# barry-mir/mixing-style-transfer

Measured on AMD Instinct MI355X. Metric: triplets/sec (10 s @ 44.1 kHz, 4-stem, bs=24), higher is better.
Workload: dtype f32

## Files before the change

mixing-style-transfer_amd/csrc/encoder.hip:

```cpp
#include "common.h"

#include <cmath>
#include <type_traits>
#include <vector>

namespace {

typedef float f32x4 __attribute__((ext_vector_type(4)));
constexpr int kConvThreads = 512;
constexpr int kConvWaves = 8;

struct FilmParams {
  const float* feats;
  const float *w0t, *b0, *w3t, *b3, *hwt, *hb;
  const float *s1, *t1, *s2, *t2;
  float* film;
  float2* aff1;
  float2* aff2;
  int Fd, H, nsub;
  float* h2;
  int B;
};

constexpr int kFilmCT = 8;
// ... 97 lines not shown
      p.aff2[((size_t)b * p.nsub + band) * 64 + c2] = make_float2(g * p.s2[band * 64 + c2], fmaf(g, p.t2[band * 64 + c2], be));
    }
  }
}

constexpr size_t film_lds_bytes(int Fd, int H) {
  return (size_t)((Fd + H) * kFilmCT + 5 * kFilmCT * 64) * sizeof(float);
}
hipError_t launch_film(const FilmParams& fp, hipStream_t st) {
  const int tiles = (fp.B + kFilmCT - 1) / kFilmCT;
  const size_t lds_h = (size_t)((fp.Fd + fp.H) * kFilmCT + 4 * kFilmCT * 64) * sizeof(float);
  const size_t lds_o = (size_t)(fp.H * kFilmCT + 5 * kFilmCT * 64) * sizeof(float);
  hipLaunchKernelGGL(film_hidden_kernel, dim3(tiles, (fp.H + 63) / 64), dim3(256), lds_h, st, fp);
  hipLaunchKernelGGL(film_head_kernel, dim3(tiles, fp.nsub * 3), dim3(256), lds_o, st, fp);
  return hipGetLastError();
}

template <int LAYER, int SUB>
struct CC;
template <int SUB>
struct CC<1, SUB> {
  static constexpr int CIN = 8, COUT = 32, NCH = 2, MT = 5, NT = 2;
  static constexpr int WIN = 5 * SUB;
  static constexpr int WPG = 20 / WIN;
  static constexpr int TROWS = SUB, TCOLS = 5 * 4 * WPG;
  static constexpr int PR = TROWS + 6, PC = TCOLS + 6;
  static constexpr int RL = PC <= 64 ? 64 : 128;
};
template <int SUB>
struct CC<2, SUB> {
  static constexpr int CIN = 32, COUT = 64, NCH = 8, MT = 4, NT = 4;
  static constexpr int WIN = 16, WPG = 1;
  static constexpr int TROWS = 8, TCOLS = 8;
  static constexpr int PR = 14, PC = 14;
  static constexpr int RL = 16;
};

template <int SUB>
struct CC<3, SUB> {
  static constexpr int CIN = 64, COUT = 32, NCH = 16, MT = 5, NT = 2;
  static constexpr int WIN = 10, WPG = 2;
  static constexpr int TROWS = 2, TCOLS = 40;
  static constexpr int PR = TROWS + 6, PC = TCOLS + 6;
  static constexpr int RL = 64;
};

template <int SUB>
struct CC<4, SUB> {
  static constexpr int CIN = 32, COUT = 64, NCH = 8, MT = 5, NT = 4;
  static constexpr int WIN = 10, WPG = 2;
  static constexpr int TROWS = 2, TCOLS = 40;
  static constexpr int PR = TROWS + 6, PC = TCOLS + 6;
  static constexpr int RL = 64;
};

struct ConvParams {
  const float* in;
  const float* wfrag;
  const float2* aff;
  float* out;
  int B, nsub;
  int in_rows, in_cols;
  int in_cstride;
  int in_bandoff;
  long long in_clipstride;
  int out_rows, out_cols;
  int tiles_r, tiles_c;
  int sets_per_band;
  float* yraw;
  mst::DetAcc* stats;
  const float* bias;
  int raw_rows, raw_cols;
  const unsigned char* mask;
  float mask_scale;
  int acc_tr, acc_tc, row_off;
  const float* f16_scale;
  const float* f16_winv;
  int pool_h;
  int clip_major;
  _Float16* yraw16;
  const float* y_scale;
  const void* in_lo;
  int cm_mels, cm_overlap;
};

typedef _Float16 h16x4 __attribute__((ext_vector_type(4)));
__device__ __forceinline__ size_t yvec(size_t unit, int t, int nvec) {
  return (unit & ~(size_t)63) * nvec + (size_t)t * 64 + (unit & 63);
}
template <int NV>
__device__ __forceinline__ void load_unit(const void* yraw, const float* y_scale, int band, size_t unit, float (&v)[NV]) {
  if (y_scale) {
    const float inv = y_scale[band * 2 + 1];
    const h16x4* s = reinterpret_cast<const h16x4*>(yraw);
#pragma unroll
    for (int t = 0; t < NV / 4; ++t) {
      const h16x4 q = s[yvec(unit, t, NV / 4)];
#pragma unroll
      for (int r = 0; r < 4; ++r) v[4 * t + r] = (float)q[r] * inv;
    }
  } else {
    const f32x4* s = reinterpret_cast<const f32x4*>(yraw);
#pragma unroll
    for (int t = 0; t < NV / 4; ++t) {
      const f32x4 q = s[yvec(unit, t, NV / 4)];
#pragma unroll
      for (int r = 0; r < 4; ++r) v[4 * t + r] = q[r];
    }
  }
}

template <int NT, int COUT>
__device__ __forceinline__ void flush_stats(double (&st)[NT][2], mst::DetAcc* stats, int band, int lane) {
#pragma unroll
  for (int n = 0; n < NT; ++n)
#pragma unroll
    for (int k = 0; k < 2; ++k) {
      double x = st[n][k];
      x += __shfl_xor(x, 16, 64);
      x += __shfl_xor(x, 32, 64);
      if (lane < 16) mst::det_add(&stats[((size_t)band * COUT + n * 16 + lane) * 2 + k], x);
      st[n][k] = 0.0;
    }
}

struct Tile {
  int valid, clip, band, tr, tc;
};

template <class F, int... I>
__device__ __forceinline__ void static_for_impl(F&& f, std::integer_sequence<int, I...>) {
  (f(std::integral_constant<int, I>{}), ...);
}
template <int N, class F>
__device__ __forceinline__ void static_for(F&& f) {
  static_for_impl(f, std::make_integer_sequence<int, N>{});
}


template <int LAYER, int SUB>
struct ConvGeom {
  using C = CC<LAYER, SUB>;
  static constexpr int WCH = 49 * C::NT * 64;
  static constexpr int NWF = (WCH / 4 + kConvThreads - 1) / kConvThreads;
  static constexpr int WBP = NWF * kConvThreads * 4;
  static constexpr int PATCH = (4 * C::PR * C::PC + 3) / 4 * 4;
  static constexpr int NPF = (4 * C::PR * C::RL + 63) / 64;
  static constexpr int NCV = C::RL >= 64 ? C::RL / 64 : 1;
};

template <int LAYER, int SUB, int MODE = 0>
__global__ __launch_bounds__(kConvThreads) void conv_kernel(const ConvParams p) {
  using C = CC<LAYER, SUB>;
  using GEO = ConvGeom<LAYER, SUB>;
  static_assert(MODE == 0 || (MODE == 1 && LAYER <= 2) || (MODE == 2 && LAYER == 3) || (MODE == 3 && LAYER == 4),
                "raw modes: forward layers, conv2 dgrad, conv2 strip");
  constexpr bool GEO1 = LAYER == 1 || LAYER >= 3;
  constexpr int MT = C::MT, NT = C::NT, NCH = C::NCH, PR = C::PR, PC = C::PC, RL = C::RL;
  constexpr int WBP = GEO::WBP, PATCH = GEO::PATCH, NWF = GEO::NWF, NPF = GEO::NPF, NCV = GEO::NCV;
  constexpr bool BL = LAYER == 2;
  constexpr int NPFK = BL ? 16 : NPF;
  constexpr int NPIECE = NPFK + NWF, PPT = (NPIECE + 48) / 49;
  extern __shared__ __attribute__((aligned(16))) float smem[];
  const int tid = threadIdx.x, lane = tid & 63;
  const int wave = __builtin_amdgcn_readfirstlane(tid >> 6);
  float* wbuf = smem;
// ... 266 lines not shown
            st[n][0] += (double)v, st[n][1] += (double)v * (double)v;
            const int tr8 = row >> 3, rr = row & 7, tc8 = col >> 3, cc8 = col & 7;
            const int lane8 = 16 * (((rr >> 2) << 1) | (cc8 >> 2)) + j, e8 = 4 * (rr & 3) + (cc8 & 3);
            yplane[(((((size_t)tr8 * p.acc_tc + tc8) * NT + n) * 4 + (e8 >> 2)) * 64 + lane8) * 4 + (e8 & 3)] = v;
          }
        }
      }
    }
    if (MODE == 2 && chunk == NCH - 1 && cur.valid) {
      const int j = lane & 15, g = lane >> 4;
#pragma unroll
      for (int n = 0; n < NT; ++n) {
        const int ch = n * 16 + j;
        float* ob = p.out + (((size_t)cur.clip * p.nsub + cur.band) * C::COUT + ch) * (size_t)p.raw_rows * p.raw_cols;
        const unsigned char* mb = p.mask ? p.mask + (((size_t)cur.clip * p.nsub + cur.band) * C::COUT + ch) * (size_t)p.raw_rows * p.raw_cols
                                         : nullptr;
#pragma unroll
        for (int e = 0; e < 4 * MT; ++e) {
          const int wv = e / C::WIN, pos = e % C::WIN;
          const int row = C::TROWS * cur.tr + pos / 5, col = C::TCOLS * cur.tc + 5 * (C::WPG * g + wv) + pos % 5;
          if (row < p.raw_rows && col < p.raw_cols) {
            const size_t o = (size_t)row * p.raw_cols + col;
            float v = acc[e >> 2][n][e & 3];
            if (mb) v = mb[o] ? v * p.mask_scale : 0.f;
            ob[o] = v;
          }
        }
      }
    }
    if (MODE == 0 && chunk == NCH - 1 && cur.valid) {
      const int j = lane & 15, g = lane >> 4;
      const float2* aff = p.aff + ((size_t)cur.clip * p.nsub + cur.band) * C::COUT;
#pragma unroll
      for (int n = 0; n < NT; ++n) {
        const int ch = n * 16 + j;
        const float2 ac = aff[ch];
        if constexpr (LAYER == 1) {
#pragma unroll
          for (int wv = 0; wv < C::WPG; ++wv) {
            float m = 0.f;
#pragma unroll
            for (int pos = 0; pos < C::WIN; ++pos) {
              const int e = wv * C::WIN + pos;
              m = fmaxf(m, fmaf(acc[e >> 2][n][e & 3], ac.x, ac.y));
            }
            const int pc = 4 * C::WPG * cur.tc + C::WPG * g + wv;
            if (pc < p.out_cols)
              p.out[((((size_t)cur.clip * p.nsub + cur.band) * C::COUT + ch) * p.out_rows + cur.tr) * p.out_cols + pc] = m;
          }
        } else {
          float m = 0.f;
          if constexpr (TS) {
            float m0 = 0.f, m1 = 0.f;
#pragma unroll
            for (int r = 0; r < 4; ++r) {
              m0 = fmaxf(m0, fmaxf(fmaf(acc[0][n][r], ac.x, ac.y), fmaf(acc[1][n][r], ac.x, ac.y)));
              m1 = fmaxf(m1, fmaxf(fmaf(acc[2][n][r], ac.x, ac.y), fmaf(acc[3][n][r], ac.x, ac.y)));
            }
            m0 = fmaxf(m0, __shfl_xor(m0, 32, 64));
            m1 = fmaxf(m1, __shfl_xor(m1, 32, 64));
            m = (g >> 1) ? m1 : m0;
          } else {
#pragma unroll
            for (int t = 0; t < MT; ++t)
#pragma unroll
              for (int r = 0; r < 4; ++r) m = fmaxf(m, fmaf(acc[t][n][r], ac.x, ac.y));
          }
          const int pr = 2 * cur.tr + (g >> 1), pc = 2 * cur.tc + (g & 1);
          if (pr < p.out_rows && pc < p.out_cols)
            p.out[(((size_t)cur.clip * p.nsub + cur.band) * C::COUT + ch) * p.out_rows * p.out_cols +
                  (size_t)pr * p.out_cols + pc] = m;
        }
      }
    }
  }
#ifdef MST_TRACE
  if (MODE == 0 && LAYER == 2 && lane == 0 && p.yraw) {
    float* o = p.yraw + (blockIdx.x * kConvWaves + wave) * 8;
    for (int i = 0; i < 5; ++i) o[i] = (float)trc[i];
    o[5] = (float)(clock64() - trc_start);
  }
#endif
  if ((MODE == 1 || MODE == 3) && st_band >= 0) flush_stats<NT, C::COUT>(st, p.stats, st_band, lane);
}

template <int SUB, int MODE = 0, int LAY = 0>
__global__ __launch_bounds__(kConvThreads) void conv1_resident_kernel(const ConvParams p) {
  using C = CC<1, SUB>;
  constexpr int MT = C::MT, NT = C::NT, PR = C::PR, PC = C::PC;
  static_assert(C::RL == 64, "resident conv1 expects one loader row per instruction");
  static_assert(LAY == 0 || PR == 8, "the channel-minor loader maps lane bits 1..3 to the 8 patch rows");
  constexpr int WCH = 49 * NT * 64;
  constexpr int WBP = ConvGeom<1, SUB>::WBP;
  constexpr int CHS = PR * PC;
  constexpr int PATCH = 8 * CHS;
  constexpr int NPF = LAY == 0 ? 8 * PR : (PC + 3) / 4;
  extern __shared__ __attribute__((aligned(16))) float smem[];
  const int tid = threadIdx.x, lane = tid & 63;
  const int wave = __builtin_amdgcn_readfirstlane(tid >> 6);
  float* wres = smem;
  float* pbuf = smem + 2 * WCH + wave * PATCH;
  constexpr bool DYN = MODE == 0;
  constexpr int kTickets = 16;
  __shared__ unsigned tickets[kTickets];
#ifdef MST_TRACE
  long long trc[5] = {0, 0, 0, 0, 0};
  const long long trc_start = clock64();
#endif

  const int G = gridDim.x;
  const int wg = mst::xcd_remap(blockIdx.x, G);
  const int total_sets = (p.clip_major ? (p.B + p.clip_major - 1) / p.clip_major : 1) * p.nsub * p.sets_per_band;
  const int s_begin = (int)((long long)wg * total_sets / G), s_end = (int)((long long)(wg + 1) * total_sets / G);
  const int tpb = p.tiles_r * p.tiles_c;

  auto decode = [&](int s) __attribute__((always_inline)) {
    Tile t;
    int ti;
    if (p.clip_major) {
      const int ngrp = (p.B + p.clip_major - 1) / p.clip_major;
      const int gb = min(s / p.sets_per_band, ngrp * p.nsub - 1);
      const int idx = (s - gb * p.sets_per_band) * kConvWaves + wave;
      const int grp = gb / p.nsub, c0 = grp * p.clip_major;
      t.band = gb - grp * p.nsub;
      t.valid = (s < s_end) && idx < min(p.clip_major, p.B - c0) * tpb;
      const int cl = t.valid ? idx / tpb : 0;
      t.clip = c0 + cl;
      ti = t.valid ? idx - cl * tpb : 0;
    } else {
      t.band = min(s / p.sets_per_band, p.nsub - 1);
      const int idx = (s - t.band * p.sets_per_band) * kConvWaves + wave;
      t.valid = (s < s_end) && idx < p.B * tpb;
      t.clip = t.valid ? idx / tpb : 0;
      ti = t.valid ? idx - t.clip * tpb : 0;
    }
    t.tc = ti / p.tiles_r;
    t.tr = ti - t.tc * p.tiles_r;
    return t;
  };

  const int kq = lane >> 4, ai = lane & 15, ag = ai >> 2, areg = ai & 3;
  int abase[MT];
#pragma unroll
  for (int t = 0; t < MT; ++t) {
    const int e = 4 * t + areg, wv = e / C::WIN, pos = e % C::WIN;
    abase[t] = kq * CHS + (pos / 5) * PC + 5 * (C::WPG * ag + wv) + pos % 5;
  }

  typename std::conditional<LAY == 0, float, f32x4>::type pf[NPF];
  unsigned long long rowmask = 0;
  bool col_ok = false;
  int coff = 0, nrow0 = 0, nvalid = 0;
  const float* nsrc = p.in;
  bool nfast = false;
  __amdgpu_buffer_rsrc_t nrsrc = __builtin_amdgcn_make_buffer_rsrc(const_cast<float*>(p.in), 0, 0, 0x00020000);
  unsigned nsoff = 0, nvoff = 0;
  static_assert(WBP - WCH >= 4, "the chunk pitch leaves at least 16 zero bytes behind the weights");
  const float* const zero16 = p.wfrag + WCH;
  const int lr = (lane >> 1) & 7, lhalf = lane & 1, lfq = lane >> 4;
  const unsigned frame_bytes = (unsigned)p.cm_mels * 32u;
  auto prefetch_setup = [&](const Tile& t) __attribute__((always_inline)) {
    nrow0 = C::TROWS * t.tr - 3;
    nvalid = t.valid;
    rowmask = 0;
    if constexpr (LAY == 0) {
      const int col0 = C::TCOLS * t.tc - 3, cin = col0 + lane;
// ... 2334 lines not shown
          for (int c = 0; c < 4; ++c) {
            const float a = low ? dyl[((c * 4 + (lane >> 5)) * 64 + (lane & 31)) * 4 + e] : dyl[((c * 4 + (e >> 2)) * 64 + lane) * 4 + (e & 3)];
            acc[c][KF] = __builtin_amdgcn_mfma_f32_16x16x4f32(a, b, acc[c][KF], 0, 0, 0);
          }
        }
      }
    }
    stage(buf ^ 1, pfs, dqs, pms);
    __syncthreads();
  };
  for (int s = s_begin; s < s_end; s += 2) {
    body(s, 0, pfA, dqA, pmA, pfB, dqB, pmB);
    if (s + 1 < s_end) body(s + 1, 1, pfB, dqB, pmB, pfA, dqA, pmA);
  }
  flush(cur_band, cur_chunk);
}

#include "encoder_f16train.inc"

__global__ void sums_to_dbn_kernel(const mst::DetAcc* sums, float* dbn, int n, const float* unscale) {
  const int i = blockIdx.x * blockDim.x + threadIdx.x;
  const double u = unscale ? (double)unscale[1] : 1.0;
  if (i < n) dbn[i] = (float)(mst::det_get(sums[2 * i + 1]) * u), dbn[n + i] = (float)(mst::det_get(sums[2 * i]) * u);
}

__global__ void dfilm_finish_kernel(const mst::DetAcc* acc, float* dfilm, int n192, int goff, int boff, int cout,
                                    const float* unscale) {
  const int i = blockIdx.x * blockDim.x + threadIdx.x;
  if (i >= n192 / 192 * 2 * cout) return;
  const int cb = i / (2 * cout), r = i % (2 * cout);
  const int slot = r < cout ? goff + r : boff + (r - cout);
  const double u = unscale ? (double)unscale[1] : 1.0;
  dfilm[(size_t)cb * 192 + slot] += (float)(mst::det_get(acc[(size_t)cb * 192 + slot]) * u);
}

__global__ void det_to_float_kernel(const mst::DetAcc* acc, float* out, long long n, const float* unscale) {
  const long long i = (long long)blockIdx.x * blockDim.x + threadIdx.x;
  const double u = unscale ? (double)unscale[1] : 1.0;
  if (i < n) out[i] = (float)(mst::det_get(acc[i]) * u);
}

__global__ void conv_fragments_kernel(const float* w, float* f, int nsub, int cout, int cin, int wchp) {
  const int nt = cout / 16, nch = cin / 4;
  const long long total = (long long)nsub * nch * 49 * nt * 64;
  const long long i = (long long)blockIdx.x * blockDim.x + threadIdx.x;
  if (i >= total) return;
  const int lane = (int)(i & 63);
  long long r = i >> 6;
  const int n = (int)(r % nt);
  r /= nt;
  const int tap = (int)(r % 49);
  r /= 49;
  const int ch = (int)(r % nch), b = (int)(r / nch);
  const int co = n * 16 + (lane & 15), ci = 4 * ch + (lane >> 4);
  f[((size_t)b * nch + ch) * wchp + ((size_t)tap * nt + n) * 64 + lane] = w[(((size_t)b * cout + co) * cin + ci) * 49 + tap];
}

__global__ void dgrad_fragments_kernel(const float* w, float* f, int nsub, int wchp) {
  const long long total = (long long)nsub * 16 * 49 * 2 * 64;
  const long long i = (long long)blockIdx.x * blockDim.x + threadIdx.x;
  if (i >= total) return;
  const int lane = (int)(i & 63);
  long long r = i >> 6;
  const int n = (int)(r % 2);
  r /= 2;
  const int tap = (int)(r % 49);
  r /= 49;
  const int ch = (int)(r % 16), b = (int)(r / 16);
  const int co = 4 * ch + (lane >> 4), ci = n * 16 + (lane & 15);
  f[((size_t)b * 16 + ch) * wchp + ((size_t)tap * 2 + n) * 64 + lane] = w[(((size_t)b * 64 + co) * 32 + ci) * 49 + (48 - tap)];
}

template <int LAYER, int SUB>
hipError_t launch_conv(const ConvParams& cp, int grid, hipStream_t st) {
  using GEO = ConvGeom<LAYER, SUB>;
  const size_t lds = (size_t)(2 * GEO::WBP + kConvWaves * GEO::PATCH) * sizeof(float);
  static unsigned long long attr_set = 0;
  if (mst::first_use_on_device(attr_set)) {
    hipError_t e = hipFuncSetAttribute(reinterpret_cast<const void*>(conv_kernel<LAYER, SUB>),
                                       hipFuncAttributeMaxDynamicSharedMemorySize, (int)lds);
    if (e != hipSuccess) return e;
  }
  hipLaunchKernelGGL((conv_kernel<LAYER, SUB>), dim3(grid), dim3(kConvThreads), lds, st, cp);
  return hipGetLastError();
}

}

extern "C" {

int mst_encoder_create(mst_encoder** out, const mst_encoder_config* cfg, const mst_encoder_weights* w) {
  MST_REQUIRE(out, "mst_encoder_create: NULL out");
  *out = nullptr;
  MST_REQUIRE(cfg && w, "mst_encoder_create: NULL config/weights");
  const int ns = cfg->n_subbands;
  MST_REQUIRE(ns >= 1 && cfg->split_size >= 4 && cfg->overlap >= 1 && cfg->n_mels >= cfg->split_size,
              "mst_encoder_create: bad band split (n_mels=%d split=%d overlap=%d n_sub=%d)", cfg->n_mels,
              cfg->split_size, cfg->overlap, ns);
  MST_REQUIRE((ns - 1) * cfg->overlap + cfg->split_size <= cfg->n_mels, "mst_encoder_create: sub-bands exceed n_mels");
  const int sub = cfg->split_size / 10 > 1 ? cfg->split_size / 10 : 1;
  MST_REQUIRE(sub <= 2 || (size_t)(392 * 32 + 8 * (cfg->split_size + 6) * kGenPC) * sizeof(float) <= 160 * 1024,
              "mst_encoder_create: split_size=%d (first-pool height %d) exceeds the generic conv1 kernel's LDS (split_size <= 68)",
              cfg->split_size, sub);
  MST_REQUIRE(cfg->attn_hidden == 256, "mst_encoder_create: attn_hidden must be 256 (got %d)", cfg->attn_hidden);
  MST_REQUIRE(cfg->feature_dim >= 1 && cfg->film_hidden >= 1 && cfg->embed_dim >= 1, "mst_encoder_create: bad dims");
  MST_REQUIRE(film_lds_bytes(cfg->feature_dim, cfg->film_hidden) <= 64 * 1024,
              "mst_encoder_create: feature_dim=%d + film_hidden=%d exceed the FiLM kernels' LDS tile (8 clips x (feature_dim + film_hidden) "
              "floats + 10 KB <= 64 KB)", cfg->feature_dim, cfg->film_hidden);
  for (const float* const* q = &w->conv1_w; q <= &w->proj_b; ++q)
    MST_REQUIRE(*q != nullptr, "mst_encoder_create: NULL weight pointer");
  mst_encoder* e = new mst_encoder();
  e->cfg = *cfg;
  e->sub = sub;
  e->H1 = cfg->split_size / sub;
  e->FD = e->H1 / 4;
  e->C = 64 * ns * e->FD;
  MST_REQUIRE(e->FD >= 1 && e->C % 4 == 0, "mst_encoder_create: bad pooled geometry");
  int dev = 0;
  hipDeviceProp_t prop;
  if (hipGetDevice(&dev) == hipSuccess && hipGetDeviceProperties(&prop, dev) == hipSuccess && prop.multiProcessorCount > 0)
    e->num_cus = prop.multiProcessorCount;
  const int H = cfg->film_hidden, Fd = cfg->feature_dim, A = cfg->attn_hidden, E = cfg->embed_dim, C = e->C;
  auto fold = [&](const float* cb, const float* bw, const float* bb, const float* mean, const float* var, int n,
                  std::vector<float>& s, std::vector<float>& t) {
    s.resize(n), t.resize(n);
    for (int i = 0; i < n; ++i) {
      const double sc = (double)bw[i] / std::sqrt((double)var[i] + (double)cfg->bn_eps);
      s[i] = (float)sc;
      t[i] = (float)(sc * ((double)cb[i] - (double)mean[i]) + (double)bb[i]);
    }
  };
  std::vector<float> s1, t1, s2, t2;
  fold(w->conv1_b, w->bn1_w, w->bn1_b, w->bn1_mean, w->bn1_var, ns * 32, s1, t1);
  fold(w->conv2_b, w->bn2_w, w->bn2_b, w->bn2_mean, w->bn2_var, ns * 64, s2, t2);
  auto f1 = conv_fragments(w->conv1_w, ns, 32, 8, ConvGeom<1, 2>::WBP);
  auto f2 = conv_fragments(w->conv2_w, ns, 64, 32, ConvGeom<2, 2>::WBP);
  auto w0t = transpose(w->mlp0_w, H, Fd), w3t = transpose(w->mlp3_w, H, H), hwt = transpose(w->head_w, ns * 192, H);
  MST_REQUIRE(E % 16 == 0, "mst_encoder_create: embed_dim must be a multiple of 16 (got %d)", E);
  std::vector<float> pfrag((size_t)(C / 4) * (E / 16) * 64);
  for (int s = 0; s < C / 4; ++s)
    for (int n = 0; n < E / 16; ++n)
      for (int lane = 0; lane < 64; ++lane)
        pfrag[((size_t)s * (E / 16) + n) * 64 + lane] = w->proj_w[(size_t)(n * 16 + (lane & 15)) * C + 4 * s + (lane >> 4)];
  std::vector<float> af((size_t)(C / 4) * (A / 16) * 64);
  for (int s = 0; s < C / 4; ++s)
    for (int n = 0; n < A / 16; ++n)
      for (int lane = 0; lane < 64; ++lane)
        af[((size_t)s * (A / 16) + n) * 64 + lane] = w->att0_w[(size_t)(n * 16 + (lane & 15)) * C + 4 * s + (lane >> 4)];
  std::vector<int> wex1((size_t)ns * 32), wex2((size_t)ns * 64);
  std::vector<float> winv1((size_t)ns * 32), winv2((size_t)ns * 64);
  for (int b = 0; b < ns; ++b) {
    for (int co = 0; co < 32; ++co) {
      float mx = 0.f;
      for (int i = 0; i < 392; ++i) mx = std::max(mx, fabsf(w->conv1_w[((size_t)b * 32 + co) * 392 + i]));
      wex1[(size_t)b * 32 + co] = f16_weight_exponent(mx);
      winv1[(size_t)b * 32 + co] = ldexpf(1.0f, -wex1[(size_t)b * 32 + co]);
    }
    for (int co = 0; co < 64; ++co) {
      float mx = 0.f;
      for (int i = 0; i < 1568; ++i) mx = std::max(mx, fabsf(w->conv2_w[((size_t)b * 64 + co) * 1568 + i]));
      wex2[(size_t)b * 64 + co] = f16_weight_exponent(mx);
      winv2[(size_t)b * 64 + co] = ldexpf(1.0f, -wex2[(size_t)b * 64 + co]);
    }
  }
  std::vector<_Float16> f16((size_t)ns * kF16Steps * 2 * 2 * 64 * 8);
  for (int b = 0; b < ns; ++b)
// ... 277 lines not shown
        cp.clip_major = std::max(1, std::min(B, env ? atoi(env) : 1));
        cp.sets_per_band = (cp.clip_major * cp.tiles_r * cp.tiles_c + kConvWaves - 1) / kConvWaves;
      }
      const int g = std::min(grid, (cp.clip_major ? (B + cp.clip_major - 1) / cp.clip_major : 1) * ns * cp.sets_per_band);
      constexpr size_t lds = (size_t)(2 * 49 * C::NT * 64 + kConvWaves * 8 * C::PR * C::PC) * sizeof(float);
      static unsigned long long attr_set = 0;
      if (mst::first_use_on_device(attr_set)) {
        err = hipFuncSetAttribute(reinterpret_cast<const void*>(conv1_resident_kernel<2>),
                                  hipFuncAttributeMaxDynamicSharedMemorySize, (int)lds);
        if (err == hipSuccess)
          err = hipFuncSetAttribute(reinterpret_cast<const void*>(conv1_resident_kernel<2, 0, 1>),
                                    hipFuncAttributeMaxDynamicSharedMemorySize, (int)lds);
        if (err != hipSuccess) return mst::fail(MST_EHIP, "conv1 attribute failed: %s", hipGetErrorString(err));
      }
#ifdef MST_TRACE
      static float* trace_buf = nullptr;
      if (!trace_buf) (void)hipMalloc(&trace_buf, 256 * kConvWaves * 8 * sizeof(float));
      cp.yraw = trace_buf;
#endif
      if (lay == MST_LOGMEL_CM32) hipLaunchKernelGGL((conv1_resident_kernel<2, 0, 1>), dim3(g), dim3(kConvThreads), lds, st, cp);
      else hipLaunchKernelGGL((conv1_resident_kernel<2>), dim3(g), dim3(kConvThreads), lds, st, cp);
#ifdef MST_TRACE
      {
        static int calls = 0;
        if (++calls == 10) {
          (void)hipDeviceSynchronize();
          std::vector<float> h(256 * kConvWaves * 8);
          (void)hipMemcpy(h.data(), trace_buf, h.size() * sizeof(float), hipMemcpyDeviceToHost);
          for (int w = 0; w < kConvWaves; ++w) {
            double a[6] = {0, 0, 0, 0, 0, 0};
            for (int b = 0; b < g; ++b)
              for (int i = 0; i < 6; ++i) a[i] += h[(b * kConvWaves + w) * 8 + i] / g;
            fprintf(stderr, "trace wave %d: tiles %.1f  k-steps %.0f (%.0f per tile)  wait for the patch loads %.0f (%.0f)  stage %.0f (%.0f)  barriers %.0f  total %.0f\n",
                    w, a[4], a[0], a[0] / a[4], a[1], a[1] / a[4], a[2], a[2] / a[4], a[3], a[5]);
          }
        }
      }
#endif
      err = hipGetLastError();
    } else {
      err = e->sub == 2 ? launch_conv<1, 2>(cp, g, st) : launch_conv<1, 1>(cp, g, st);
    }
    if (err != hipSuccess) return mst::fail(MST_EHIP, "conv1 launch failed: %s", hipGetErrorString(err));
  }
  mark(2);
  {
    ConvParams cp{};
    cp.in = pool1, cp.wfrag = e->w2frag, cp.aff = aff2, cp.out = pool_in, cp.B = B, cp.nsub = ns;
    cp.in_rows = e->H1, cp.in_cols = L.W1;
    cp.in_cstride = e->H1 * L.W1;
    cp.in_bandoff = 32 * e->H1 * L.W1;
    cp.in_clipstride = (long long)ns * 32 * e->H1 * L.W1;
    cp.out_rows = e->FD, cp.out_cols = L.W2;
    cp.tiles_r = (e->FD + 1) / 2;
    cp.tiles_c = (L.W2 + 1) / 2;
    cp.sets_per_band = (B * cp.tiles_r * cp.tiles_c + kConvWaves - 1) / kConvWaves;
    const int g = std::min(grid, ns * cp.sets_per_band);
    hipError_t err;
    if (e->conv1_f16x3 >= 2) {
      constexpr size_t lds = (size_t)(kF16Steps * 4 * 2 * 64 + kConvWaves * 2 * 14 * 14) * 16;
      static unsigned long long attr = 0;
      if (mst::first_use_on_device(attr)) {
        err = hipFuncSetAttribute(reinterpret_cast<const void*>(conv2_f16x3_kernel<3>),
                                  hipFuncAttributeMaxDynamicSharedMemorySize, (int)lds);
        if (err == hipSuccess)
          err = hipFuncSetAttribute(reinterpret_cast<const void*>(conv2_f16x3_kernel<1>),
                                    hipFuncAttributeMaxDynamicSharedMemorySize, (int)lds);
        if (err != hipSuccess) return mst::fail(MST_EHIP, "conv2 f16x3 attribute failed: %s", hipGetErrorString(err));
      }
      cp.f16_scale = reinterpret_cast<const float*>(ws + L.f16scale);
      cp.f16_winv = e->f16_winv2;
      const h16x8* ih = reinterpret_cast<const h16x8*>(ws + L.pool1_h16);
      const h16x8* il = reinterpret_cast<const h16x8*>(ws + L.pool1_l16);
      const h16x8* wf = reinterpret_cast<const h16x8*>(e->w2frag16);
      if (e->conv1_f16x3 == 3) hipLaunchKernelGGL((conv2_f16x3_kernel<1>), dim3(g), dim3(kConvThreads), lds, st, cp, ih, il, wf);
      else hipLaunchKernelGGL((conv2_f16x3_kernel<3>), dim3(g), dim3(kConvThreads), lds, st, cp, ih, il, wf);
      err = hipGetLastError();
    } else {
#ifdef MST_TRACE
      static float* trace_buf2 = nullptr;
      if (!trace_buf2) (void)hipMalloc(&trace_buf2, 256 * kConvWaves * 8 * sizeof(float));
      cp.yraw = trace_buf2;
#endif
      err = launch_conv<2, 2>(cp, g, st);
#ifdef MST_TRACE
      {
        static int calls = 0;
        if (++calls == 10) {
          (void)hipDeviceSynchronize();
          std::vector<float> h(256 * kConvWaves * 8);
          (void)hipMemcpy(h.data(), trace_buf2, h.size() * sizeof(float), hipMemcpyDeviceToHost);
          for (int w = 0; w < kConvWaves; ++w) {
            double a[6] = {0, 0, 0, 0, 0, 0};
            for (int b = 0; b < g; ++b)
              for (int i = 0; i < 6; ++i) a[i] += h[(b * kConvWaves + w) * 8 + i] / g;
            fprintf(stderr, "conv2 trace wave %d: chunks %.1f  staging %.0f (%.0f per chunk)  barrier wait %.0f (%.0f)  taps %.0f (%.0f)  total %.0f\n",
                    w, a[4], a[0], a[0] / a[4], a[1], a[1] / a[4], a[2], a[2] / a[4], a[5]);
          }
        }
      }
#endif
    }
    if (err != hipSuccess) return mst::fail(MST_EHIP, "conv2 launch failed: %s", hipGetErrorString(err));
  }
  mark(3);
  {
    AttnParams ap{pool_in, e->att0frag, e->att0_b, e->att2_w, scores, B, e->C, L.W2, e->cfg.attn_hidden};
    MST_HIP_CHECK(launch_attn_scores(ap, st));
  }
  mark(4);
  {
    float* pooled = reinterpret_cast<float*>(ws + L.pooled);
    PoolParams pp{pool_in, scores, e->att2_b, pooled, e->C, L.W2, (long long)B * L.W2};
    const int slices = (e->C + 127) / 128;
    hipLaunchKernelGGL(attn_pool_kernel, dim3(B, slices), dim3(256), (size_t)((L.W2 + 3) & ~3) * sizeof(float), st, pp);
    MST_HIP_CHECK(hipGetLastError());
    ProjParams pj{pooled, e->projfrag, e->proj_b, emb, B, e->C, e->cfg.embed_dim};
    launch_proj(pj, st);
    MST_HIP_CHECK(hipGetLastError());
  }
  mark(5);
  return MST_OK;
}

namespace {
struct TrainLayout {
  WsLayout base;
  size_t y1, y2, stats1, stats2, bn1, bn2, dfilm_acc, dw_acc, total;
  size_t t_pool1_h16, t_pool1_l16, t_f16scale, t_xmax, t_bscale, t_dyg1, t_dyg2, t_ys1, t_ys2;
  int tr1, tc1, tr2, tc2;
};
TrainLayout train_layout(const mst_encoder* e, int B, int frames) {
  TrainLayout T{};
  T.base = ws_layout(e, B, frames);
  const int ns = e->cfg.n_subbands;
  const bool two_row = e->sub == 2 || train_fwd16(e);
  const int tcols1 = two_row ? 40 : 80;
  T.tr1 = two_row ? e->cfg.split_size / 2 : e->H1, T.tc1 = (frames + tcols1 - 1) / tcols1;
  T.tr2 = (e->H1 + 7) / 8, T.tc2 = (T.base.W1 + 7) / 8;
  size_t o = T.base.total;
  auto take = [&](size_t bytes) {
    const size_t at = o;
    o += mst::align_up(bytes, 256);
    return at;
  };
  const size_t ybytes = e->train_f16 == 1 ? 2 : 4;
  T.y1 = take((size_t)B * ns * T.tr1 * T.tc1 * 2 * 64 * 20 * ybytes);
  T.y2 = take((size_t)B * ns * T.tr2 * T.tc2 * 4 * 64 * 16 * ybytes);
  T.stats1 = take((size_t)(ns * 32 * 2 + 1) * sizeof(mst::DetAcc));
  T.stats2 = take((size_t)(ns * 64 * 2 + 1) * sizeof(mst::DetAcc));
  T.bn1 = take((size_t)ns * 32 * 8);
  T.bn2 = take((size_t)ns * 64 * 8);
  T.dfilm_acc = take((size_t)B * ns * 192 * sizeof(mst::DetAcc));
  T.dw_acc = take((size_t)ns * 64 * 1568 * sizeof(mst::DetAcc));
  const size_t f = train_fwd16(e) ? 1 : 0, fb = train_bwd16(e) ? 1 : 0;
  T.t_pool1_h16 = take(f * (size_t)B * ns * 32 * e->H1 * T.base.W1 * 2);
  T.t_pool1_l16 = take((e->train_f16 == 2 ? 1 : 0) * (size_t)B * ns * 32 * e->H1 * T.base.W1 * 2);
  T.t_f16scale = take(f * (size_t)B * ns * 2 * 4);
  T.t_xmax = take(f * (size_t)B * 4);
  T.t_ys1 = take((e->train_f16 == 1 ? 1 : 0) * (size_t)ns * 2 * 4);
  T.t_ys2 = take((e->train_f16 == 1 ? 1 : 0) * (size_t)ns * 2 * 4);
  T.t_bscale = take(fb * 16);
  const size_t cgs = (size_t)((B + 7) / 8);
  const size_t hl = e->train_f16 == 2 ? 2 : 1;
  T.t_dyg1 = take(fb * hl * (size_t)ns * cgs * T.tr1 * T.tc1 * 2 * 20 * 64 * 16);
  T.t_dyg2 = take(fb * hl * (size_t)ns * cgs * T.tr2 * T.tc2 * 4 * 16 * 64 * 16);
  T.total = o;
// ... 774 lines not shown
```

Measured before the change: 2818.

## Add row-strip tiled conv2 kernel for two-row pooled output shape

Adds a conv2 kernel specialised for the case where the pooled output has two rows (FD==2, H1==10). Each wave computes a strip of one output row by four pooled columns from a 10x22 input patch, and a folded 14x14 variant handles leftover columns. Per-kind tap masks skip MFMAs on rows that fall outside the output. The goal is to avoid the padding and wasted work of the generic 8x8 tile on this short output. The cost is a larger, more specialised code path selected by shape, with an environment variable to fall back to the old kernel.

```diff
diff --git a/mixing-style-transfer_amd/csrc/encoder.hip b/mixing-style-transfer_amd/csrc/encoder.hip
--- a/mixing-style-transfer_amd/csrc/encoder.hip
+++ b/mixing-style-transfer_amd/csrc/encoder.hip
@@ -203,6 +203,7 @@
   const float* y_scale;
   const void* in_lo;
   int cm_mels, cm_overlap;
+  int rt_blocks, rt_fold, rt_pair_sets;
 };
 
 typedef _Float16 h16x4 __attribute__((ext_vector_type(4)));
@@ -635,6 +636,217 @@
   }
 #endif
   if ((MODE == 1 || MODE == 3) && st_band >= 0) flush_stats<NT, C::COUT>(st, p.stats, st_band, lane);
+}
+
+struct RowTiles {
+  static constexpr int PC = 22;
+  static constexpr int PR = 10;
+  static constexpr int FR = 14, FC = 14;
+  static constexpr int CP = 304;
+  static constexpr int PATCH = 4 * CP;
+};
+
+__global__ __launch_bounds__(kConvThreads) void conv2_rows_kernel(const ConvParams p) {
+  using C = CC<2, 2>;
+  using GEO = ConvGeom<2, 2>;
+  using R = RowTiles;
+  constexpr int MT = 4, NT = C::NT, NCH = C::NCH, PC = R::PC, CP = R::CP;
+  constexpr int WBP = GEO::WBP, NWF = GEO::NWF;
+  constexpr int NPFK = 16;
+  constexpr int NPIECE = NPFK + NWF, PPT = (NPIECE + 48) / 49;
+  static_assert(MT == C::MT && (R::PR - 1) * PC + PC <= 256 && R::FR * 16 <= 256, "4 pieces of 64 lanes cover a channel of either kind");
+  static_assert((R::FR - 1) * PC + R::FC <= CP && CP % 32 == 16, "channel pitch, see RowTiles");
+  static_assert((size_t)(2 * WBP + kConvWaves * R::PATCH) * sizeof(float) <= 160 * 1024, "conv2_rows_kernel must fit one CU's LDS");
+  extern __shared__ __attribute__((aligned(16))) float smem[];
+  const int tid = threadIdx.x, lane = tid & 63;
+  const int wave = __builtin_amdgcn_readfirstlane(tid >> 6);
+  float* wbuf = smem;
+  float* pbuf = smem + 2 * WBP + wave * R::PATCH;
+
+  const int G = gridDim.x;
+  const int wg = mst::xcd_remap(blockIdx.x, G);
+  const int total_sets = p.nsub * p.sets_per_band;
+  const int my_sets = wg < total_sets ? (total_sets - wg + G - 1) / G : 0;
+  const int nq = my_sets * NCH;
+  const int fold_blk = p.out_cols >> 2;
+
+  struct RTile {
+    int valid, clip, band, blk, kind;
+  };
+  auto decode = [&](int q) __attribute__((always_inline)) {
+    const int s = wg + (q / NCH) * G;
+    RTile t;
+    t.band = min(s / p.sets_per_band, p.nsub - 1);
+    const int sb = s - t.band * p.sets_per_band;
+    const bool fold = sb >= p.rt_pair_sets;
+    const int idx = fold ? (sb - p.rt_pair_sets) * kConvWaves + wave : sb * 4 + (wave & 3);
+    const int per = fold ? p.rt_fold : p.rt_blocks;
+    t.valid = q < nq && idx < p.B * per;
+    t.clip = t.valid ? idx / per : 0;
+    t.blk = fold ? fold_blk : (t.valid ? idx - t.clip * per : 0);
+    t.kind = fold ? 2 : wave >> 2;
+    return t;
+  };
+
+  const int kq = lane >> 4, ai = lane & 15;
+  const float* const ap_pair = pbuf + kq * CP + ai;
+  const float* const ap_fold = pbuf + kq * CP + 4 * (ai >> 3) * PC + (ai & 7);
+  const float* ap = ap_pair;
+
+  f32x4 wreg[NWF];
+  float pf[NPFK];
+  __amdgpu_buffer_rsrc_t nrsrc = __builtin_amdgcn_make_buffer_rsrc(const_cast<float*>(p.in), 0, 0, 0x00020000);
+  __amdgpu_buffer_rsrc_t nwrsrc = __builtin_amdgcn_make_buffer_rsrc(const_cast<float*>(p.wfrag), 0, 0, 0x00020000);
+  unsigned nvoff[4] = {0x80000000u, 0x80000000u, 0x80000000u, 0x80000000u}, nsoff = 0;
+  int nsaddr[4] = {-1, -1, -1, -1};
+
+  auto prefetch_setup = [&](int q, const RTile& t) __attribute__((always_inline)) {
+    const int chunk = q % NCH;
+    const float* src = p.in + (size_t)t.clip * p.in_clipstride + (size_t)t.band * p.in_bandoff + (size_t)(4 * chunk) * p.in_cstride;
+    const float* wsrc = p.wfrag + ((size_t)t.band * NCH + chunk) * WBP;
+    nrsrc = __builtin_amdgcn_make_buffer_rsrc(const_cast<float*>(src), 0, (unsigned)(4 * p.in_cstride) * 4u, 0x00020000);
+    nwrsrc = __builtin_amdgcn_make_buffer_rsrc(const_cast<float*>(wsrc), 0, (unsigned)WBP * 4u, 0x00020000);
+    if (chunk == 0) {
+      const bool fold = t.kind == 2;
+      const int row0 = (t.kind == 1 ? 4 : 0) - 3, col0 = 16 * t.blk - 3;
+      const int rbase = max(row0, 0), cbase = max(col0, 0);
+      nsoff = (unsigned)(rbase * p.in_cols + cbase) * 4u;
+      int ln = lane;
+      asm volatile("" : "+v"(ln));
+#pragma unroll
+      for (int j = 0; j < 4; ++j) {
+        const int e = ln + 64 * j;
+        const int r = fold ? e >> 4 : e / PC, c = fold ? e & 15 : e % PC;
+        const bool in_patch = fold ? (r < R::FR && c < R::FC) : r < R::PR;
+        const int rin = row0 + r, cin = col0 + c;
+        const bool ok = t.valid && in_patch && rin >= 0 && rin < p.in_rows && cin >= 0 && cin < p.in_cols;
+        nvoff[j] = ok ? (unsigned)((rin - rbase) * p.in_cols + (cin - cbase)) * 4u : 0x80000000u;
+        nsaddr[j] = in_patch ? r * PC + c : -1;
+      }
+    }
+  };
+  auto prefetch_piece = [&](int i) __attribute__((always_inline)) {
+    if (i < NPFK) {
+      pf[i] = __builtin_bit_cast(float, __builtin_amdgcn_raw_buffer_load_b32(nrsrc, nvoff[i & 3], nsoff + (unsigned)((i >> 2) * p.in_cstride) * 4u, 0));
+    } else if (i < NPIECE) {
+      wreg[i - NPFK] = __builtin_bit_cast(f32x4, __builtin_amdgcn_raw_buffer_load_b128(nwrsrc, (unsigned)tid * 16u, (unsigned)(kConvThreads * (i - NPFK)) * 16u, 0));
+    }
+  };
+
+  f32x4 acc[MT][NT];
+  RTile cur{}, nxt{};
+  nxt = decode(0);
+  if (nq > 0) {
+    prefetch_setup(0, nxt);
+#pragma unroll
+    for (int i = 0; i < NPIECE; ++i) prefetch_piece(i);
+  }
+#ifdef MST_TRACE
+  long long trc[5] = {0, 0, 0, 0, 0};
+  const long long trc_start = clock64();
+#endif
+  for (int q = 0; q < nq; ++q) {
+    float* wb = wbuf + (q & 1) * WBP;
+#ifdef MST_TRACE
+    const long long tq0 = clock64();
+#endif
+#pragma unroll
+    for (int i = 0; i < NWF; ++i) reinterpret_cast<f32x4*>(wb)[tid + kConvThreads * i] = wreg[i];
+#pragma unroll
+    for (int i = 0; i < NPFK; ++i)
+      if (nsaddr[i & 3] >= 0) pbuf[(i >> 2) * CP + nsaddr[i & 3]] = pf[i];
+#ifdef MST_TRACE
+    asm volatile("s_waitcnt lgkmcnt(0)" ::: "memory");
+    const long long tq1 = clock64();
+#endif
+    __syncthreads();
+#ifdef MST_TRACE
+    const long long tq2 = clock64();
+    trc[0] += tq1 - tq0, trc[1] += tq2 - tq1, trc[4] += 1;
+#endif
+    cur = nxt;
+    if ((q + 1) % NCH == 0) nxt = decode(q + 1);
+    prefetch_setup(q + 1, nxt);
+    const int chunk = q % NCH;
+    if (chunk == 0) {
+      ap = cur.kind == 2 ? ap_fold : ap_pair;
+#pragma unroll
+      for (int t = 0; t < MT; ++t)
+#pragma unroll
+        for (int n = 0; n < NT; ++n) acc[t][n] = f32x4{0.f, 0.f, 0.f, 0.f};
+    }
+    {
+      float a[2][MT], b[2][NT];
+#pragma unroll
+      for (int t = 0; t < MT; ++t) a[0][t] = ap[t * PC];
+#pragma unroll
+      for (int n = 0; n < NT; ++n) b[0][n] = wb[n * 64 + lane];
+      auto taps = [&](auto LO_, auto HI_, auto MASK_) __attribute__((always_inline)) {
+        constexpr int LO = decltype(LO_)::value, HI = decltype(HI_)::value, MASK = decltype(MASK_)::value;
+#pragma unroll
+        for (int tap = LO; tap < HI; ++tap) {
+          const int cu = tap & 1, nx = cu ^ 1;
+          const int off = ((tap + 1) / 7) * PC + ((tap + 1) % 7);
+#pragma unroll
+          for (int i = 0; i < MT * NT; ++i) {
+            const int t = i / NT, n = i % NT;
+            if (!((MASK >> t) & 1)) acc[t][n] = __builtin_amdgcn_mfma_f32_16x16x4f32(a[cu][t], b[cu][n], acc[t][n], 0, 0, 0);
+            if (tap + 1 < 49) {
+              if (i < NT) b[nx][i] = wb[((tap + 1) * NT + i) * 64 + lane];
+              else if (i < MT + NT) a[nx][i - NT] = ap[(i - NT) * PC + off];
+            }
+            if (i >= MT + NT && i - (MT + NT) < PPT) prefetch_piece(tap * PPT + (i - (MT + NT)));
+            __builtin_amdgcn_sched_barrier(0);
+          }
+        }
+      };
+      using std::integral_constant;
+      using I0 = integral_constant<int, 0>;
+      using I7 = integral_constant<int, 7>;
+      using I14 = integral_constant<int, 14>;
+      using I21 = integral_constant<int, 21>;
+      using I42 = integral_constant<int, 42>;
+      using I49 = integral_constant<int, 49>;
+      if (cur.kind == 0) {
+        taps(I0{}, I7{}, integral_constant<int, 0b0111>{});
+        taps(I7{}, I14{}, integral_constant<int, 0b0011>{});
+        taps(I14{}, I21{}, integral_constant<int, 0b0001>{});
+      } else {
+        taps(I0{}, I21{}, I0{});
+      }
+      taps(I21{}, I42{}, I0{});
+      if (cur.kind == 1) taps(I42{}, I49{}, integral_constant<int, 0b1000>{});
+      else taps(I42{}, I49{}, I0{});
+    }
+#ifdef MST_TRACE
+    trc[2] += clock64() - tq2;
+#endif
+    if (chunk == NCH - 1 && cur.valid) {
+      const int j = lane & 15, g = lane >> 4;
+      const float2* aff = p.aff + ((size_t)cur.clip * p.nsub + cur.band) * C::COUT;
+      const int pr = cur.kind == 2 ? g >> 1 : cur.kind;
+      const int pc = 4 * cur.blk + (cur.kind == 2 ? g & 1 : g);
+#pragma unroll
+      for (int n = 0; n < NT; ++n) {
+        const int ch = n * 16 + j;
+        const float2 ac = aff[ch];
+        float m = 0.f;
+#pragma unroll
+        for (int t = 0; t < MT; ++t)
+#pragma unroll
+          for (int r = 0; r < 4; ++r) m = fmaxf(m, fmaf(acc[t][n][r], ac.x, ac.y));
+        if (pc < p.out_cols)
+          p.out[(((size_t)cur.clip * p.nsub + cur.band) * C::COUT + ch) * p.out_rows * p.out_cols + (size_t)pr * p.out_cols + pc] = m;
+      }
+    }
+  }
+#ifdef MST_TRACE
+  if (lane == 0 && p.yraw) {
+    float* o = p.yraw + (blockIdx.x * kConvWaves + wave) * 8;
+    for (int i = 0; i < 5; ++i) o[i] = (float)trc[i];
+    o[5] = (float)(clock64() - trc_start);
+  }
+#endif
 }
 
 template <int SUB, int MODE = 0, int LAY = 0>
@@ -3135,6 +3347,18 @@
     if (e != hipSuccess) return e;
   }
   hipLaunchKernelGGL((conv_kernel<LAYER, SUB>), dim3(grid), dim3(kConvThreads), lds, st, cp);
+  return hipGetLastError();
+}
+
+hipError_t launch_conv2_rows(const ConvParams& cp, int grid, hipStream_t st) {
+  const size_t lds = (size_t)(2 * ConvGeom<2, 2>::WBP + kConvWaves * RowTiles::PATCH) * sizeof(float);
+  static unsigned long long attr_set = 0;
+  if (mst::first_use_on_device(attr_set)) {
+    hipError_t e = hipFuncSetAttribute(reinterpret_cast<const void*>(conv2_rows_kernel),
+                                       hipFuncAttributeMaxDynamicSharedMemorySize, (int)lds);
+    if (e != hipSuccess) return e;
+  }
+  hipLaunchKernelGGL(conv2_rows_kernel, dim3(grid), dim3(kConvThreads), lds, st, cp);
   return hipGetLastError();
 }
 
@@ -3578,7 +3802,17 @@
       if (!trace_buf2) (void)hipMalloc(&trace_buf2, 256 * kConvWaves * 8 * sizeof(float));
       cp.yraw = trace_buf2;
 #endif
-      err = launch_conv<2, 2>(cp, g, st);
+      const char* tiles_env = getenv("MST_CONV2_TILES");
+      if (e->FD == 2 && e->H1 == 10 && !(tiles_env && !strcmp(tiles_env, "8x8"))) {
+        const int rem = L.W2 % 4;
+        cp.rt_blocks = L.W2 / 4 + (rem == 3);
+        cp.rt_fold = rem == 1 || rem == 2;
+        cp.rt_pair_sets = (B * cp.rt_blocks + 3) / 4;
+        cp.sets_per_band = cp.rt_pair_sets + (B * cp.rt_fold + kConvWaves - 1) / kConvWaves;
+        err = launch_conv2_rows(cp, std::min(grid, ns * cp.sets_per_band), st);
+      } else {
+        err = launch_conv<2, 2>(cp, g, st);
+      }
 #ifdef MST_TRACE
       {
         static int calls = 0;
```

New measurement: 2848, median of 6. 1.01x the previous value.
